# rubund/gnuais

Measured on AMD Instinct MI355X. Metric: Msamples/s demodulated (N-channel batch, full chain), higher is better.
Workload: dtype f32 FIR on int16 samples; u32 PLL/HDLC/CRC; 1 GPU; C3: 16384 ch x 48000 samples @48 kHz per GPU, full chain incl. HDLC/CRC-16; channels_per_gpu=16384, samples_per_channel=48000, parallelism=channels sharded over 1 GPU(s), one process per GPU, no collectives

## Files before the change

gnuais_amd/csrc/hdlc_crc.hip:

```cpp
#include <hip/hip_runtime.h>
#include <stdint.h>

#include "kernels.h"

namespace gnuais {

enum { ST_SKURR = 1, ST_PREAMBLE = 2, ST_STARTSIGN = 3, ST_DATA = 4, ST_STOPSIGN = 5 };

constexpr uint32_t CAND_VALID = 0x10000u;
constexpr int PACK_MAX = PACK_STRIDE;

__global__ void hdlc_reset_kernel(uint32_t *__restrict__ ctl, int N)
{
    const int c = blockIdx.x * blockDim.x + threadIdx.x;
    if (c >= N) return;
    ctl[c] = ST_SKURR;
    ctl[(size_t) N + c] = 0;
    ctl[(size_t) 2 * N + c] = 0;
    ctl[(size_t) 3 * N + c] = 0;
    ctl[(size_t) 4 * N + c] = 0;
    ctl[(size_t) 5 * N + c] = 0;
}

__global__ void hdlc_fsm_reset_kernel(uint32_t *__restrict__ ctl, int N)
{
    const int c = blockIdx.x * blockDim.x + threadIdx.x;
    if (c >= N) return;
    ctl[c] = ST_SKURR;
    ctl[(size_t) N + c] = 0;
    ctl[(size_t) 4 * N + c] = 0;
}

__device__ __forceinline__ uint32_t lowmask(int k)
{
    return k >= 32 ? ~0u : ((1u << k) - 1u);
}
__device__ __forceinline__ int ctz32(uint32_t v)
{
    return v ? __ffs((int) v) - 1 : 32;
}
__device__ __forceinline__ int clz32(uint32_t v)
{
    return v ? __clz((int) v) : 32;
}

__global__ __launch_bounds__(64) __attribute__((amdgpu_waves_per_eu(7, 8))) void hdlc_deframe_kernel(
    const uint32_t *__restrict__ segbits, const uint32_t *__restrict__ segcnt,
    uint32_t *__restrict__ ctl, uint32_t *__restrict__ cand, uint32_t *__restrict__ cand_first,
    uint32_t *__restrict__ cand_count, int32_t *__restrict__ counters,
    uint32_t *__restrict__ flags, int N, int n_seg, int seg_words, int K)
{
    __builtin_amdgcn_s_setprio(3);
    const int cg = blockIdx.x * blockDim.x + threadIdx.x;
    const bool live = cg < N;
    const size_t c = (size_t) (live ? cg : N - 1), n_ = (size_t) N;

    const uint32_t c0 = ctl[c];
    int state = c0 & 7, nstartsign = (c0 >> 3) & 15, antallpreamble = (c0 >> 7) & 15;
    int antallenner = (c0 >> 11) & 7, bitstuff = (c0 >> 14) & 1;
    uint32_t last = (c0 >> 15) & 1;
    int bufferpos = (c0 >> 16) & 511;
    uint32_t cur = ctl[n_ + c];
    const uint32_t seen0 = ctl[2 * n_ + c], seenhi0 = ctl[5 * n_ + c];
    uint32_t nstart = ctl[3 * n_ + c];
    int rawpos = (int) ctl[4 * n_ + c];
    int lost2 = 0;

    const bool open0 = (state == ST_DATA || state == ST_STOPSIGN);
    const uint32_t first = nstart - (open0 ? 1u : 0u);
    uint32_t *rec = cand + ((size_t) c * K + (open0 ? (nstart - 1) % (uint32_t) K : 0u)) * CAND_WORDS;
    bool rec_ok = open0;

    uint32_t seenbase = seen0;

#define HDLC_RESET()                                                                    \
    do { state = ST_SKURR; nstartsign = 0; antallpreamble = 0; antallenner = 0;        \
         last = 0; bitstuff = 0; bufferpos = 0; } while (0)

    extern __shared__ uint32_t lds_pack[];
    const int tpb = (int) blockDim.x, tx = (int) threadIdx.x;
    const uint32_t *__restrict__ rows = segbits + c * (size_t) n_seg * (size_t) PACK_STRIDE;
    uint32_t pf[PACK_MAX];
    int pf_cnt = live ? (int) segcnt[c * (size_t) n_seg] : 0;
#pragma unroll
    for (int q = 0; q < PACK_MAX / 4; ++q) {
        const uint4 v = reinterpret_cast<const uint4 *>(rows)[q];
        pf[4 * q] = v.x; pf[4 * q + 1] = v.y; pf[4 * q + 2] = v.z; pf[4 * q + 3] = v.w;
    }

    for (int seg = 0; seg < n_seg; ++seg) {
        int tile_end = pf_cnt;
        if (tile_end > seg_words * 32) tile_end = seg_words * 32;
#pragma unroll
        for (int q = 0; q < PACK_MAX; ++q) lds_pack[q * tpb + tx] = pf[q];
        lds_pack[PACK_MAX * tpb + tx] = 0;
        if (seg + 1 < n_seg) {
            const uint32_t *__restrict__ nrow = rows + (size_t) (seg + 1) * (size_t) PACK_STRIDE;
            pf_cnt = live ? (int) segcnt[c * (size_t) n_seg + seg + 1] : 0;
#pragma unroll
            for (int q = 0; q < PACK_MAX / 4; ++q) {
                const uint4 v = reinterpret_cast<const uint4 *>(nrow)[q];
                pf[4 * q] = v.x; pf[4 * q + 1] = v.y; pf[4 * q + 2] = v.z; pf[4 * q + 3] = v.w;
            }
        }
        int pos = 0;
#define FETCH_WINDOW()                                                                          \
        const int lw = pos >> 5, sh = pos & 31;                                                 \
        const uint32_t lo = lds_pack[lw * tpb + tx], hi = lds_pack[(lw + 1) * tpb + tx];        \
        const uint32_t W = sh ? ((lo >> sh) | (hi << (32 - sh))) : lo;   \
        const int nv = (tile_end - pos < 32) ? tile_end - pos : 32

        while (__any(pos < tile_end)) {
            while (__any(pos < tile_end && state == ST_SKURR)) {
                if (pos < tile_end && state == ST_SKURR) {
                    FETCH_WINDOW();
                    const uint32_t vm = lowmask(nv);
                    const uint32_t A = W ^ ((W << 1) | last);
                    const uint32_t B2 = A & (A << 1), B4 = B2 & (B2 << 2), B8 = B4 & (B4 << 4);
                    const uint32_t B15 = B8 & (B8 << 7);
                    const int t = ctz32(~A);
                    const int need = 14 - antallpreamble;
                    const uint32_t C = lowmask(t) & ~lowmask(need > 0 ? need : 0);
                    const uint32_t TR = (B15 | C) & ~W & vm;
                    if (TR) {
                        pos += ctz32(TR) + 1;
                        state = ST_PREAMBLE;
                        antallpreamble = 0;
                        last = 0;
                    } else {
                        pos += nv;
                        last = (W >> (nv - 1)) & 1u;
                        const int ap = (t >= nv) ? antallpreamble + nv : clz32(~(A << (32 - nv)));
                        antallpreamble = ap > 15 ? 15 : ap;
                    }
                }
            }
            while (__any(pos < tile_end && state != ST_SKURR && state != ST_DATA)) {
                if (pos < tile_end && state != ST_SKURR && state != ST_DATA) {
                    FETCH_WINDOW();
                    int k = 0;
                    if (state == ST_STOPSIGN) {
                        const uint32_t x = W & 1u;
                        const int nb = bufferpos - 6 - 16;
                        if (x == 0 && nb > 0) {
                            if (rec_ok) {
                                rec[CAND_HDR + (rawpos >> 5)] = cur;
                                const uint32_t eb = seenbase + (uint32_t) pos;
                                const uint32_t ebhi = (seenhi0 + (eb < seen0 ? 1u : 0u)) & 31u;
                                rec[1] = eb;
                                rec[0] = (uint32_t) nb | CAND_VALID | ((uint32_t) rawpos << 17) | (ebhi << 27);
                            }
                        } else {
                            ++lost2;
                            if (rec_ok) {
                                rec[CAND_HDR + (rawpos >> 5)] = cur;
                                rec[0] = (uint32_t) rawpos << 17;
                            }
                        }
                        HDLC_RESET();
                        last = x;
                        k = 1;
                    } else if (state != ST_PREAMBLE && state != ST_STARTSIGN) {
                        HDLC_RESET();
                        last = W & 1u;
                        k = 1;
                    } else {
                        if (state == ST_PREAMBLE && nstartsign == 0) {
                            const uint32_t A = W ^ ((W << 1) | last);
                            int t = ctz32(~A);
                            if (t > nv) t = nv;
                            if (t > 0) {
                                antallpreamble = antallpreamble + t > 15 ? 15 : antallpreamble + t;
                                last = (W >> (t - 1)) & 1u;
                                k = t;
                            }
                            if (k < nv) {
                                const uint32_t x0 = (W >> k) & 1u;
                                nstartsign = x0 ? 3 : 1;
                                last = x0;
                                ++k;
                            }
                        }
                        if (k < nv && nstartsign != 0) {
                            const int R = 7 - nstartsign;
                            const int avail = nv - k;
                            int L = ctz32(~(W >> k));
                            if (L > avail) L = avail;
                            if (L >= R + 1) {
                                HDLC_RESET(); nstartsign = 1; last = 1; k += R + 1;
                            } else if (L < avail) {
                                if (L == R) {
                                    state = ST_DATA; nstartsign = 1; antallenner = 0; antallpreamble = 0;
                                    bufferpos = 0; cur = 0; rawpos = 0; bitstuff = 0; last = 0;
                                    rec_ok = (nstart - first) < (uint32_t) K;
                                    rec = cand + ((size_t) c * K + nstart % (uint32_t) K) * CAND_WORDS;
                                    if (rec_ok) rec[0] = 0; else flags[1] = 1;
                                    ++nstart;
                                } else if (L == R - 1) {
                                    HDLC_RESET(); nstartsign = 1; last = 0;
                                } else {
                                    HDLC_RESET(); last = 0;
                                }
                                k += L + 1;
                            } else {
                                nstartsign += L;
                                if (nstartsign >= 6) { state = ST_STARTSIGN; antallpreamble = 0; }
                                last = 1;
                                k += L;
                            }
                        }
                    }
                    pos += k;
                }
            }
            while (__any(pos < tile_end && state == ST_DATA)) {
                if (pos < tile_end && state == ST_DATA) {
                    FETCH_WINDOW();
                    if (bitstuff) {
                        const uint32_t x = W & 1u;
                        if (x) {
                            state = ST_STOPSIGN;
                        } else {
                            if ((rawpos & 31) == 31) {
                                if (rec_ok) rec[CAND_HDR + (rawpos >> 5)] = cur;
                                cur = 0;
                            }
// ... 9 lines not shown
                        if (nw > 32 - m) nw = 32 - m;
                        if (nw > room) nw = room;
                        const int nvE = nw + m;
                        const uint32_t vmE = lowmask(nvE);
                        const uint32_t E = ((W << m) | lowmask(m)) & vmE;
                        const uint32_t X1 = E & (E >> 1), X2 = X1 & (X1 >> 2);
                        const uint32_t R5 = X2 & (E >> 4);
                        const uint32_t S5 = R5 & ~(E << 1);
                        const uint32_t P5 = S5 << 4;
                        const uint32_t nx = E >> 1, kn = vmE >> 1;
                        const uint32_t END5 = P5 & nx & kn;
                        const uint32_t STF5 = P5 & ~nx & kn;
                        const uint32_t PND5 = P5 & ~kn;
                        int nraw, stored;
                        if (END5) {
                            const int pe = ctz32(END5);
                            nraw = pe + 1 - m;
                            stored = nraw - __popc(STF5 & lowmask(pe));
                        } else {
                            nraw = nw;
                            stored = nw - __popc(STF5);
                        }
                        {
                            const uint32_t sb = W & lowmask(nraw);
                            const int bsh = rawpos & 31;
                            const uint64_t t64 = (uint64_t) sb << bsh;
                            cur |= (uint32_t) t64;
                            if (bsh + nraw >= 32) {
                                if (rec_ok) rec[CAND_HDR + (rawpos >> 5)] = cur;
                                cur = (uint32_t) (t64 >> 32);
                            }
                            rawpos += nraw;
                        }
                        bufferpos += stored;
                        if (END5) {
                            pos += nraw + 1;
                            state = ST_STOPSIGN;
                            antallenner = 0;
                            last = 1;
                        } else {
                            pos += nraw;
                            const uint32_t xl = (W >> (nraw - 1)) & 1u;
                            if (bufferpos >= 449) {
                                if (rec_ok) rec[0] = 0;
                                HDLC_RESET();
                                last = xl;
                            } else if (PND5) {
                                bitstuff = 1;
                                antallenner = 0;
                                last = 1;
                            } else {
                                const int r = clz32(~(E << (32 - nvE)));
                                last = xl;
                                antallenner = r > 0 ? r - 1 : 0;
                            }
                        }
                    }
                }
            }
        }
#undef FETCH_WINDOW
        seenbase += (uint32_t) tile_end;
    }
#undef HDLC_RESET

    if (live) {
        ctl[c] = (uint32_t) state | ((uint32_t) nstartsign << 3) | ((uint32_t) antallpreamble << 7) |
                 ((uint32_t) antallenner << 11) | ((uint32_t) bitstuff << 14) | (last << 15) |
                 ((uint32_t) bufferpos << 16);
        ctl[n_ + c] = cur;
        ctl[2 * n_ + c] = seenbase;
        ctl[5 * n_ + c] = seenhi0 + (seenbase < seen0 ? 1u : 0u);
        ctl[3 * n_ + c] = nstart;
        ctl[4 * n_ + c] = (uint32_t) rawpos;
        const bool open1 = (state == ST_DATA || state == ST_STOPSIGN);
        const uint32_t limit = nstart - (open1 ? 1u : 0u);
        cand_first[c] = first;
        uint32_t cnt = limit - first;
        cand_count[c] = cnt > (uint32_t) K ? (uint32_t) K : cnt;
        if (lost2) counters[2 * n_ + c] += lost2;
    }
}

__global__ __launch_bounds__(256) void hdlc_crc_kernel(
    const uint32_t *__restrict__ cand, const uint32_t *__restrict__ cand_first,
    const uint32_t *__restrict__ cand_count, int32_t *__restrict__ counters,
    uint32_t *__restrict__ frames, uint32_t *__restrict__ flags, uint32_t frame_cap, int N, int K,
    uint2 *__restrict__ chunks, int n_pass)
{
    __shared__ uint32_t tab[256];
    __shared__ uint32_t pre[K3_CH + 1];
    extern __shared__ uint32_t k3_dyn[];
    uint32_t (*const stage)[HDLC_BUF_WORDS + 1] = reinterpret_cast<uint32_t (*)[HDLC_BUF_WORDS + 1]>(k3_dyn);
    uint32_t (*const rawlds)[CAND_WORDS - CAND_HDR + 1] =
        reinterpret_cast<uint32_t (*)[CAND_WORDS - CAND_HDR + 1]>(k3_dyn + 256 * (HDLC_BUF_WORDS + 1));
    __shared__ uint32_t wave_cnt[4];
    __shared__ uint32_t pass_base;
    const int tid = threadIdx.x;
    const int c_own = blockIdx.x * K3_CH + tid;

    {
        uint32_t t = (uint32_t) tid;
#pragma unroll
        for (int k = 0; k < 8; ++k) t = (t >> 1) ^ ((t & 1u) ? 0x8408u : 0u);
        tab[tid] = t;
    }
    if (tid < K3_CH) pre[tid + 1] = (c_own < N) ? cand_count[c_own] : 0u;
    __syncthreads();
    if (tid == 0) {
        uint32_t run = 0;
        pre[0] = 0;
        for (int q = 1; q <= K3_CH; ++q) { run += pre[q]; pre[q] = run; }
    }
    __syncthreads();
    const uint32_t total = pre[K3_CH];
    const size_t n_ = (size_t) N;

    int pass = 0;
    for (uint32_t i0 = 0; i0 < total; i0 += 256, ++pass) {
        const uint32_t i = i0 + (uint32_t) tid;
        bool good = false;
        uint32_t out[16];
#pragma unroll
        for (int q = 0; q < 16; ++q) out[q] = 0;
        if (i < total) {
            int lo = 0, hi = K3_CH - 1;
            while (lo < hi) {
                const int mid = (lo + hi + 1) >> 1;
                if (pre[mid] <= i) lo = mid; else hi = mid - 1;
            }
            const int c = blockIdx.x * K3_CH + lo;
            const uint32_t j = i - pre[lo];
            const uint32_t slot = (cand_first[c] + j) % (uint32_t) K;
            const uint32_t *rec = cand + ((size_t) c * K + slot) * CAND_WORDS;
            const uint32_t hdr = rec[0];
            if (hdr & CAND_VALID) {
                const int n = (int) (hdr & 0xffffu);
                const int rawlen = (int) ((hdr >> 17) & 0x3ffu);
                const int nbytes = n >> 3, buflen = nbytes + 2;
                {
                    uint32_t raw[CAND_WORDS - CAND_HDR];
#pragma unroll
                    for (int q = 0; q < CAND_WORDS - CAND_HDR; ++q) raw[q] = rec[CAND_HDR + q];
#pragma unroll
                    for (int q = 0; q < CAND_WORDS - CAND_HDR; ++q) rawlds[tid][q] = raw[q];
                    unsigned long long acc = 0;
                    uint32_t prevw = 0;
                    int fill = 0, ow = 0;
                    const int nwords = (rawlen + 31) >> 5;
#pragma unroll 1
                    for (int q = 0; q < nwords; ++q) {
                        uint32_t rw = rawlds[tid][q];
                        const int nvq = rawlen - 32 * q < 32 ? rawlen - 32 * q : 32;
                        const unsigned long long cc = ((unsigned long long) rw << 32) | prevw;
                        const uint32_t five = (uint32_t) (cc >> 31) & (uint32_t) (cc >> 30) & (uint32_t) (cc >> 29) &
                                              (uint32_t) (cc >> 28) & (uint32_t) (cc >> 27);
                        uint32_t stf = five & ~rw & (nvq >= 32 ? ~0u : (1u << nvq) - 1u);
                        prevw = rw;
                        int nout = nvq;
                        while (stf) {
                            const int pz = 31 - __clz((int) stf);
                            stf &= ~(1u << pz);
                            rw = (rw & ((1u << pz) - 1u)) | ((pz >= 31 ? 0u : rw >> (pz + 1)) << pz);
                            --nout;
                        }
                        if (nout < 32) rw &= (1u << nout) - 1u;
                        acc |= (unsigned long long) rw << fill;
                        fill += nout;
                        if (fill >= 32) {
                            if (ow <= HDLC_BUF_WORDS) stage[tid][ow] = (uint32_t) acc;
                            ++ow;
                            acc >>= 32;
                            fill -= 32;
                        }
                    }
                    if (ow <= HDLC_BUF_WORDS) stage[tid][ow] = (uint32_t) acc;
                    for (int q = ow + 1; q <= HDLC_BUF_WORDS; ++q) stage[tid][q] = 0;
                }
                uint32_t w[HDLC_BUF_WORDS];
#pragma unroll
                for (int q = 0; q < HDLC_BUF_WORDS; ++q) w[q] = stage[tid][q];
                uint32_t crc = 0xffffu;
#pragma unroll
                for (int q = 0; q < HDLC_BUF_WORDS; ++q) {
#pragma unroll
                    for (int bq = 0; bq < 4; ++bq) {
                        if (q * 4 + bq < buflen) {
                            const uint32_t byte = (w[q] >> (8 * bq)) & 0xffu;
                            crc = (crc >> 8) ^ tab[(crc ^ byte) & 0xffu];
                        }
                    }
                }
                if (crc == 0xf0b8u) {
                    good = true;
                    atomicAdd(&counters[c], 1);
                    out[0] = (uint32_t) c;
                    out[1] = rec[1];
#pragma unroll
                    for (int q = 0; q < 14; ++q) {
                        uint32_t v = 0;
                        if (q * 4 < nbytes) {
                            v = w[q];
                            const int keep = nbytes - q * 4;
                            if (keep < 4) v &= (1u << (8 * keep)) - 1u;
                        }
                        if (q == 13) v = (v & 0xffu) | ((1u | ((hdr >> 27) << 1)) << 8) | ((uint32_t) n << 16);
                        out[2 + q] = v;
                    }
                } else {
                    atomicAdd(&counters[n_ + c], 1);
                }
            }
        }
        const unsigned long long m = __ballot(good);
        const int wave = tid >> 6, lane = tid & 63;
        const uint32_t below = (uint32_t) __popcll(m & ((1ull << lane) - 1ull));
        if (lane == 0) wave_cnt[wave] = (uint32_t) __popcll(m);
        __syncthreads();
        uint32_t woff = 0, npass = 0;
#pragma unroll
        for (int q = 0; q < 4; ++q) {
            if (q < wave) woff += wave_cnt[q];
            npass += wave_cnt[q];
        }
        if (tid == 0) {
            const uint32_t base = npass ? atomicAdd(&flags[0], npass) : 0u;
            pass_base = base;
            if (chunks && pass < n_pass)
                chunks[(size_t) blockIdx.x * n_pass + pass] =
                    make_uint2(base, base >= frame_cap ? 0u : (npass < frame_cap - base ? npass : frame_cap - base));
        }
        __syncthreads();
        if (good) {
            const uint32_t idx = pass_base + woff + below;
            if (idx < frame_cap) {
                uint4 *dst = reinterpret_cast<uint4 *>(frames + (size_t) idx * 16);
                dst[0] = make_uint4(out[0], out[1], out[2], out[3]);
                dst[1] = make_uint4(out[4], out[5], out[6], out[7]);
                dst[2] = make_uint4(out[8], out[9], out[10], out[11]);
                dst[3] = make_uint4(out[12], out[13], out[14], out[15]);
            } else {
                flags[1] = 1;
            }
        }
        __syncthreads();
    }
    if (chunks)
        for (int q = pass + tid; q < n_pass; q += 256) chunks[(size_t) blockIdx.x * n_pass + q] = make_uint2(0u, 0u);
}

hipError_t launch_hdlc_deframe(const HdlcLaunch &a, hipStream_t stream)
{
    const int lpw = a.lanes_per_wave > 0 ? a.lanes_per_wave : 64;
    if (a.seg_words > PACK_MAX) return hipErrorInvalidValue;
    hipLaunchKernelGGL(hdlc_deframe_kernel, dim3((a.N + lpw - 1) / lpw), dim3(lpw),
                       (PACK_MAX + 1) * lpw * sizeof(uint32_t), stream,
                       a.segbits, a.segcnt, a.ctl, a.cand, a.cand_first, a.cand_count, a.counters,
                       a.frame_count, a.N, a.n_seg, a.seg_words, a.K);
    return hipGetLastError();
}

hipError_t launch_hdlc_crc(const HdlcLaunch &a, hipStream_t stream)
{
    constexpr size_t K3_DYN_LDS = 256 * ((HDLC_BUF_WORDS + 1) + (CAND_WORDS - CAND_HDR + 1)) * sizeof(uint32_t);
    hipLaunchKernelGGL(hdlc_crc_kernel, dim3((unsigned) ((a.N + K3_CH - 1) / K3_CH)), dim3(256), K3_DYN_LDS,
                       stream, a.cand, a.cand_first, a.cand_count, a.counters,
                       (uint32_t *) a.frames, a.frame_count, a.frame_cap, a.N, a.K, a.chunks, k3_passes(a.K_call > 0 ? a.K_call : a.K));
    return hipGetLastError();
}

hipError_t launch_hdlc_fsm_reset(uint32_t *ctl, int N, hipStream_t stream)
{
    hipLaunchKernelGGL(hdlc_fsm_reset_kernel, dim3((N + 255) / 256), dim3(256), 0, stream, ctl, N);
    return hipGetLastError();
}

hipError_t launch_hdlc_reset(uint32_t *ctl, int N, hipStream_t stream)
{
    hipLaunchKernelGGL(hdlc_reset_kernel, dim3((N + 255) / 256), dim3(256), 0, stream, ctl, N);
    return hipGetLastError();
}

}
```

gnuais_amd/csrc/hdlc_events.hip:

```cpp
#include <hip/hip_runtime.h>
#include <stdint.h>

#include "kernels.h"

namespace gnuais {

namespace {

enum { ST_SKURR = 1, ST_PREAMBLE = 2, ST_STARTSIGN = 3, ST_DATA = 4, ST_STOPSIGN = 5 };
constexpr uint32_t CAND_VALID = 0x10000u;
constexpr int EW = PACK_STRIDE;
constexpr int NONE = 1 << 20;

__device__ __forceinline__ uint32_t lowmask(int k) { return k >= 32 ? ~0u : k <= 0 ? 0u : ((1u << k) - 1u); }
__device__ __forceinline__ int ctz32(uint32_t v) { return v ? __ffs((int) v) - 1 : 32; }
__device__ __forceinline__ int clz32(uint32_t v) { return v ? __clz((int) v) : 32; }
__device__ __forceinline__ int wave_max_i(int v, int lanes, int lane)
{
#pragma unroll
    for (int o = 32; o; o >>= 1) {
        const int u = __shfl_xor(v, o);
        v = ((lane ^ o) < lanes && u > v) ? u : v;
    }
    return v;
}

}

constexpr int EV_ROWS = (EW + 2) + 4 * EW + (EW + 1);

template <int TPB>
__global__ __launch_bounds__(64) void hdlc_events_kernel(
    const uint32_t *__restrict__ segbits, const uint32_t *__restrict__ segcnt,
    uint32_t *__restrict__ ctl, uint32_t *__restrict__ cand, uint32_t *__restrict__ cand_first,
    uint32_t *__restrict__ cand_count, int32_t *__restrict__ counters,
    uint32_t *__restrict__ flags, int N, int n_seg, int seg_words, int K)
{
    __builtin_amdgcn_s_setprio(3);
    extern __shared__ uint32_t lds[];
    const int tpb = TPB > 0 ? TPB : (int) blockDim.x, tx = (int) threadIdx.x;
    const int cg = blockIdx.x * blockDim.x + threadIdx.x;
    const bool live = cg < N;
    const size_t c = (size_t) (live ? cg : N - 1), n_ = (size_t) N;
    uint32_t *const Xa = lds + tx, *const NAa = Xa + (EW + 2) * tpb, *const CBa = NAa + EW * tpb,
                   *const E6a = CBa + EW * tpb, *const SFa = E6a + EW * tpb, *const PSa = SFa + EW * tpb;
#define XW(q) Xa[((q) + 1) * tpb]

    const uint32_t c0 = ctl[c];
    int state = c0 & 7, nstartsign = (c0 >> 3) & 15, antallpreamble = (c0 >> 7) & 15;
    int antallenner = (c0 >> 11) & 7, bitstuff = (c0 >> 14) & 1;
    uint32_t last = (c0 >> 15) & 1;
    int bufferpos = (c0 >> 16) & 511;
    uint32_t cur = ctl[n_ + c];
    const uint32_t seen0 = ctl[2 * n_ + c], seenhi0 = ctl[5 * n_ + c];
    uint32_t nstart = ctl[3 * n_ + c];
    int rawpos = (int) ctl[4 * n_ + c];
    int lost2 = 0;

    const bool open0 = (state == ST_DATA || state == ST_STOPSIGN);
    const uint32_t first = nstart - (open0 ? 1u : 0u);
    uint32_t *rec = cand + ((size_t) c * K + (open0 ? (nstart - 1) % (uint32_t) K : 0u)) * CAND_WORDS;
    bool rec_ok = open0;
    uint32_t seenbase = seen0;

#define HDLC_RESET()                                                                    \
    do { state = ST_SKURR; nstartsign = 0; antallpreamble = 0; antallenner = 0;        \
         last = 0; bitstuff = 0; bufferpos = 0; } while (0)
#define ENTER_DATA()                                                                    \
    do { state = ST_DATA; nstartsign = 1; antallenner = 0; antallpreamble = 0;         \
         bufferpos = 0; cur = 0; rawpos = 0; bitstuff = 0; last = 0;                    \
         rec_ok = (nstart - first) < (uint32_t) K;                                      \
         rec = cand + ((size_t) c * K + nstart % (uint32_t) K) * CAND_WORDS;            \
         if (rec_ok) rec[0] = 0; else flags[1] = 1;                                     \
         ++nstart; } while (0)
#define RAW_APPEND(v_, n_bits_)                                                         \
    do { const uint32_t sb_ = (v_); const int nb_ = (n_bits_), bsh_ = rawpos & 31;      \
         const uint64_t t64_ = (uint64_t) sb_ << bsh_;                                  \
         cur |= (uint32_t) t64_;                                                        \
         if (bsh_ + nb_ >= 32) {                                                        \
             if (rec_ok) rec[CAND_HDR + (rawpos >> 5)] = cur;                           \
             cur = (uint32_t) (t64_ >> 32);                                             \
         }                                                                              \
         rawpos += nb_; } while (0)
#define STOP_BIT(x_, at_)                                                               \
    do { const int nb_ = bufferpos - 6 - 16;                                            \
         if ((x_) == 0 && nb_ > 0) {                                                    \
             if (rec_ok) {                                                              \
                 const uint32_t eb_ = seenbase + (uint32_t) (at_);                      \
                 const uint32_t ebhi_ = (seenhi0 + (eb_ < seen0 ? 1u : 0u)) & 31u;      \
                 rec[CAND_HDR + (rawpos >> 5)] = cur;                                   \
                 rec[1] = eb_;                                                          \
                 rec[0] = (uint32_t) nb_ | CAND_VALID | ((uint32_t) rawpos << 17) | (ebhi_ << 27); \
             }                                                                          \
         } else {                                                                       \
             ++lost2;                                                                   \
             if (rec_ok) {       \
                 rec[CAND_HDR + (rawpos >> 5)] = cur;                                   \
                 rec[0] = (uint32_t) rawpos << 17;                                      \
             }                                                                          \
         }                                                                              \
         HDLC_RESET();                                                                  \
         last = (x_); } while (0)

    auto slow_bit = [&](uint32_t x, int at) {
        int ns_v = nstartsign, bp_v = bufferpos;
        {
        int nstartsign = ns_v, bufferpos = bp_v;
        switch (state) {
        case ST_DATA:
            if (bitstuff) {
                if (x == 1) {
                    state = ST_STOPSIGN;
                } else {
                    RAW_APPEND(0u, 1);
                }
                bitstuff = 0;
            } else {
                if (x == last && x == 1) {
                    if (++antallenner == 4) { bitstuff = 1; antallenner = 0; }
                } else {
                    antallenner = 0;
                }
                RAW_APPEND(x, 1);
                if (++bufferpos >= 449) {
                    if (rec_ok) rec[0] = 0;
                    HDLC_RESET();
                }
            }
            break;
        case ST_SKURR:
            antallpreamble = (x != last) ? (antallpreamble < 15 ? antallpreamble + 1 : 15) : 0;
            if (antallpreamble > 14 && x == 0) { state = ST_PREAMBLE; antallpreamble = 0; }
            break;
        case ST_PREAMBLE:
            if (x != last && nstartsign == 0) {
                antallpreamble = antallpreamble < 15 ? antallpreamble + 1 : 15;
            } else if (x == 1) {
                if (nstartsign == 0) nstartsign = 3;
                else if (nstartsign == 5) { nstartsign = 6; antallpreamble = 0; state = ST_STARTSIGN; }
                else ++nstartsign;
            } else {
                if (nstartsign == 0) nstartsign = 1; else HDLC_RESET();
            }
            break;
        case ST_STARTSIGN:
            if (nstartsign >= 7) {
                if (x == 0) { ENTER_DATA(); nstartsign = 0; } else HDLC_RESET();
            } else if (x == 0) {
                HDLC_RESET();
            }
            ++nstartsign;
            if (nstartsign > 15) nstartsign = 15;
            break;
        case ST_STOPSIGN:
            STOP_BIT(x, at);
            break;
        default:
            HDLC_RESET();
            break;
        }
        ns_v = nstartsign; bp_v = bufferpos;
        }
        nstartsign = ns_v; bufferpos = bp_v;
        last = x;
    };

    const uint32_t *__restrict__ rows = segbits + c * (size_t) n_seg * (size_t) PACK_STRIDE;
    uint32_t pf[EW];
    int pf_cnt = 0;
    bool pf_ready = false;
    auto fetch = [&](int seg) {
        const uint32_t *__restrict__ row = rows + (size_t) seg * (size_t) PACK_STRIDE;
        {
            pf_cnt = live ? (int) segcnt[c * (size_t) n_seg + seg] : 0;
#pragma unroll
            for (int q = 0; q < EW / 4; ++q) {
                const uint4 v = reinterpret_cast<const uint4 *>(row)[q];
                pf[4 * q] = v.x; pf[4 * q + 1] = v.y; pf[4 * q + 2] = v.z; pf[4 * q + 3] = v.w;
            }
        }
        pf_ready = true;
    };

    for (int seg = 0; seg < n_seg; ++seg) {
        if (!pf_ready) fetch(seg);
        int tile_end = pf_cnt;
        if (tile_end > seg_words * 32) tile_end = seg_words * 32;

        const int m_in = (state == ST_DATA) ? (bitstuff ? 5 : (last ? antallenner + 1 : 0)) : 0;
        uint32_t prevw = (state == ST_DATA) ? (m_in ? ~0u << (32 - m_in) : 0u) : (last << 31);
        uint32_t ps = 0, nzNA = 0, nzCB = 0, nzE6 = 0;
        XW(-1) = prevw;
#pragma unroll
        for (int q = 0; q < EW; ++q) XW(q) = pf[q];
        pf_ready = false;
        if (seg + 1 < n_seg) fetch(seg + 1);
        const int nwq = __builtin_amdgcn_readfirstlane((int) wave_max_i((tile_end + 31) >> 5, tpb, tx));
        auto shl_in = [](uint32_t v, uint32_t below, int n) -> uint32_t {
            return __builtin_amdgcn_alignbit(v, below, 32 - n);
        };
        uint32_t pA = 0, pa2 = 0, pa4 = 0, pa8 = 0;
        uint32_t pu2 = prevw & (prevw << 1);
        uint32_t pt = (pu2 & (pu2 << 2)) & (prevw << 4);
#pragma unroll
        for (int q = 0; q < EW; ++q) {
            if (q >= nwq) {
                XW(q) = 0; NAa[q * tpb] = 0; CBa[q * tpb] = 0; E6a[q * tpb] = 0; SFa[q * tpb] = 0; PSa[q * tpb] = ps;
                continue;
            }
            const uint32_t vm = lowmask(tile_end - 32 * q);
            const uint32_t xw = XW(q) & vm;
            const uint32_t A = (xw ^ shl_in(xw, prevw, 1)) & vm;
            const uint32_t a2 = A & shl_in(A, pA, 1), a4 = a2 & shl_in(a2, pa2, 2), a8 = a4 & shl_in(a4, pa4, 4);
            const uint32_t a15 = a8 & shl_in(a8, pa8, 7);
            const uint32_t u2 = xw & shl_in(xw, prevw, 1), u4 = u2 & shl_in(u2, pu2, 2);
            const uint32_t t5 = u4 & shl_in(xw, prevw, 4);
            const uint32_t na = ~A & vm, cb = a15 & ~xw & vm;
            const uint32_t e6 = u4 & shl_in(u2, pu2, 4) & vm;
            const uint32_t sf = shl_in(t5, pt, 1) & ~xw & vm;
            XW(q) = xw;
            NAa[q * tpb] = na;
            CBa[q * tpb] = cb;
            E6a[q * tpb] = e6;
            SFa[q * tpb] = sf;
            PSa[q * tpb] = ps;
            ps += (uint32_t) __popc(sf);
            nzNA |= (na < 1u ? na : 1u) << q;
            nzCB |= (cb < 1u ? cb : 1u) << q;
            nzE6 |= (e6 < 1u ? e6 : 1u) << q;
            pA = A; pa2 = a2; pa4 = a4; pa8 = a8; pu2 = u2; pt = t5;
            prevw = xw;
        }
        XW(EW) = 0;
        PSa[EW * tpb] = ps;

        auto first_set = [&](const uint32_t *arr, uint32_t nz, int p) -> int {
            if (p >= tile_end) return NONE;
            const int q = p >> 5;
            const uint32_t m = arr[q * tpb] & (~0u << (p & 31));
            if (m) return 32 * q + ctz32(m);
            const uint32_t rest = q >= 31 ? 0u : nz & (~0u << (q + 1));
            if (!rest) return NONE;
            const int q2 = ctz32(rest);
            return 32 * q2 + ctz32(arr[q2 * tpb]);
        };
        auto bit_at = [&](int p) -> uint32_t { return (XW(p >> 5) >> (p & 31)) & 1u; };
        auto window = [&](int p) -> uint32_t {
            const int q = p >> 5, sh = p & 31;
            const uint32_t lo = XW(q), hi = XW(q + 1 <= EW ? q + 1 : EW);
            return sh ? ((lo >> sh) | (hi << (32 - sh))) : lo;
        };
        auto stuffed = [&](int a, int b) -> int {
            if (b <= a) return 0;
            const int qa = a >> 5, qb = b >> 5;
            int n = (int) PSa[qb * tpb] - (int) PSa[qa * tpb];
            n -= __popc(SFa[qa * tpb] & lowmask(a & 31));
            if (qb < EW) n += __popc(SFa[qb * tpb] & lowmask(b & 31));
            return n;
        };

        int pos = 0;
        int rs = -1;
        bool hunt0 = true;
        bool slow = false;

        auto hunt = [&]() {
            int trig = NONE;
            if (rs < 0 && hunt0) {
                const int t0 = first_set(NAa, nzNA, 0);
                int k0 = 14 - antallpreamble;
                if (k0 < 0) k0 = 0;
                const int lim = t0 < tile_end ? t0 : tile_end;
                if (k0 < lim && bit_at(k0)) ++k0;
                if (k0 < lim) trig = k0;
                const int cb = first_set(CBa, nzCB, 0);
                if (cb < trig) trig = cb;
            } else {
                const int from = rs + 15 > pos ? rs + 15 : pos;
                trig = first_set(CBa, nzCB, from);
            }
            if (trig < tile_end) {
                state = ST_PREAMBLE;
                antallpreamble = 0;
                last = 0;
                pos = trig + 1;
            } else {
                int lastna = -1;
                for (uint32_t nz = nzNA; nz;) {
                    const int q = 31 - clz32(nz);
                    const uint32_t m = NAa[q * tpb];
                    lastna = 32 * q + 31 - clz32(m);
                    break;
                }
                int ap;
                if (rs < 0 && hunt0) ap = lastna < 0 ? antallpreamble + tile_end : tile_end - 1 - lastna;
                else {
                    const int since = tile_end - 1 - rs, run = tile_end - 1 - lastna;
                    ap = since < run ? since : run;
                }
                antallpreamble = ap > 15 ? 15 : ap;
                last = bit_at(tile_end - 1);
                pos = tile_end;
            }
        };

        while (__any(pos < tile_end)) {
            if (pos < tile_end) {
                if (state == ST_SKURR && !slow) hunt();
                if (state == ST_PREAMBLE && nstartsign == 0 && pos < tile_end && !slow) {
                    const int j = first_set(NAa, nzNA, pos);
                    if (j >= tile_end) {
                        const int ap = antallpreamble + (tile_end - pos);
                        antallpreamble = ap > 15 ? 15 : ap;
                        last = bit_at(tile_end - 1);
                        pos = tile_end;
                    } else {
                        const int ap = antallpreamble + (j - pos);
                        antallpreamble = ap > 15 ? 15 : ap;
                        const uint32_t xj = bit_at(j);
                        nstartsign = xj ? 3 : 1;
                        last = xj;
                        pos = j + 1;
                    }
                }
                if (((state == ST_PREAMBLE && nstartsign != 0) || state == ST_STARTSIGN) && pos < tile_end && !slow) {
                    const uint32_t W = window(pos);
                    const int avail = tile_end - pos < 32 ? tile_end - pos : 32;
                    const int R = 7 - nstartsign;
                    int Lr = ctz32(~W);
                    if (Lr > avail) Lr = avail;
                    if (R < 0) {
                        slow = true;
                    } else if (Lr >= R + 1) {
                        HDLC_RESET(); nstartsign = 1; last = 1;
                        rs = pos + R; hunt0 = false;
                        pos += R + 1;
                    } else if (Lr < avail) {
                        if (Lr == R) {
                            ENTER_DATA();
                            pos += Lr + 1;
                        } else if (Lr == R - 1) {
                            HDLC_RESET(); nstartsign = 1; last = 0;
                            rs = pos + Lr; hunt0 = false;
                            pos += Lr + 1;
                        } else {
                            HDLC_RESET(); last = 0;
                            rs = pos + Lr; hunt0 = false;
                            pos += Lr + 1;
                        }
                    } else {
                        nstartsign += Lr;
                        if (nstartsign >= 6) { state = ST_STARTSIGN; antallpreamble = 0; }
                        last = 1;
                        pos += Lr;
                    }
                }
                if (state == ST_DATA && pos < tile_end && !slow) {
                    const int e6 = first_set(E6a, nzE6, pos);
                    const int e = e6 < tile_end ? e6 : tile_end;
                    const int stored = (e - pos) - stuffed(pos, e);
                    if (bufferpos + stored >= 449) {
                        int need = 449 - bufferpos, p = pos, t = pos;
                        for (;;) {
                            const int q = p >> 5;
                            const int we = (32 * (q + 1) < e) ? 32 * (q + 1) : e;
                            uint32_t m = ~SFa[q * tpb] & (~0u << (p & 31)) & lowmask(we - 32 * q);
                            const int n = __popc(m);
                            if (n >= need) {
                                for (int k = 1; k < need; ++k) m &= m - 1;
                                t = 32 * q + ctz32(m);
                                break;
                            }
                            need -= n;
                            p = we;
                        }
                        if (rec_ok) rec[0] = 0;
                        const uint32_t xt = bit_at(t);
                        HDLC_RESET();
                        last = xt;
                        rs = t; hunt0 = false;
                        pos = t + 1;
                    } else {
                        for (int p = pos; p < e;) {
                            const int sh = p & 31;
                            const int take = (32 - sh < e - p) ? 32 - sh : e - p;
                            RAW_APPEND((XW(p >> 5) >> sh) & lowmask(take), take);
                            p += take;
                        }
                        bufferpos += stored;
                        if (e6 < tile_end) {
                            state = ST_STOPSIGN;
                            antallenner = 0;
                            bitstuff = 0;
                            last = 1;
                            pos = e6 + 1;
                        } else {
                            int r;
                            if (tile_end >= 8) {
                                r = clz32(~(window(tile_end - 8) << 24));
                            } else {
                                r = clz32(~((XW(0) << (32 - tile_end)) | (XW(-1) >> tile_end)));
                            }
                            last = bit_at(tile_end - 1);
                            if (r >= 5) { bitstuff = 1; antallenner = 0; }
                            else { bitstuff = 0; antallenner = r > 0 ? r - 1 : 0; }
                            pos = tile_end;
                        }
                    }
                }
                if (state == ST_STOPSIGN && pos < tile_end && !slow) {
                    const uint32_t x = bit_at(pos);
                    STOP_BIT(x, pos);
                    rs = pos; hunt0 = false;
                    pos += 1;
                }
                if (pos < tile_end && (slow || state < ST_SKURR || state > ST_STOPSIGN)) {
                    const int st0 = state;
                    const uint32_t x = bit_at(pos);
                    slow_bit(x, pos);
                    if (state == ST_SKURR && st0 != ST_SKURR) { rs = pos; hunt0 = false; }
                    if (state != st0) slow = false;
                    pos += 1;
                }
                if (state == ST_SKURR && !slow && pos < tile_end) hunt();
            }
        }
        seenbase += (uint32_t) tile_end;
    }
#undef XW
#undef HDLC_RESET
#undef ENTER_DATA
#undef RAW_APPEND
#undef STOP_BIT

    if (live) {
        ctl[c] = (uint32_t) state | ((uint32_t) nstartsign << 3) | ((uint32_t) antallpreamble << 7) |
                 ((uint32_t) antallenner << 11) | ((uint32_t) bitstuff << 14) | (last << 15) |
                 ((uint32_t) bufferpos << 16);
        ctl[n_ + c] = cur;
        ctl[2 * n_ + c] = seenbase;
        ctl[5 * n_ + c] = seenhi0 + (seenbase < seen0 ? 1u : 0u);
        ctl[3 * n_ + c] = nstart;
        ctl[4 * n_ + c] = (uint32_t) rawpos;
        const bool open1 = (state == ST_DATA || state == ST_STOPSIGN);
        const uint32_t limit = nstart - (open1 ? 1u : 0u);
        cand_first[c] = first;
        uint32_t cnt = limit - first;
        cand_count[c] = cnt > (uint32_t) K ? (uint32_t) K : cnt;
        if (lost2) counters[2 * n_ + c] += lost2;
    }
}

hipError_t launch_hdlc_events(const HdlcLaunch &a, hipStream_t stream)
{
    if (a.seg_words > PACK_STRIDE) return hipErrorInvalidValue;
    const int lpw = a.lanes_per_wave >= 1 && a.lanes_per_wave <= 64 ? a.lanes_per_wave : 64;
    const dim3 grid((a.N + lpw - 1) / lpw), block(lpw);
    const size_t lds = EV_ROWS * lpw * sizeof(uint32_t);
#define EV_LAUNCH(T)                                                                                                  \
    hipLaunchKernelGGL(hdlc_events_kernel<T>, grid, block, lds, stream, a.segbits, a.segcnt, a.ctl, a.cand, a.cand_first, \
                       a.cand_count, a.counters, a.frame_count, a.N, a.n_seg, a.seg_words, a.K)
    switch (lpw) {
    case 8: EV_LAUNCH(8); break;
    case 16: EV_LAUNCH(16); break;
    case 32: EV_LAUNCH(32); break;
    case 64: EV_LAUNCH(64); break;
    default: EV_LAUNCH(0); break;
    }
#undef EV_LAUNCH
    return hipGetLastError();
}

}
```

gnuais_amd/csrc/kernels.h:

```cpp
#pragma once
#include <hip/hip_runtime.h>
#include <stdint.h>

#include "fir_plan.h"

namespace gnuais {

struct FirLaunch : FirThresholds {
    const int16_t *x;
    const int16_t *hist;
    uint32_t *sgn;
    float *dump;
    int *maxval;
    int16_t *hist_out;
    int *maxval_next;
    const float *d_taps;
    float te[64];
    int N, L;
    int NT, NE, d;
    float ctaps[48];
    const float *te_mem;
    int map;
    int max_segments = 0;
    const struct MfmaTaps *mfma = nullptr;
};
int launch_fir_sign_quantum(int NC);
hipError_t launch_fir_sign(const FirLaunch &a, hipStream_t stream);
int launch_fir_sign_pk_quantum(int NC);
struct alignas(16) MfmaTaps { int a[3][3][64][4]; int k0; };
void fir_sign_mfma_pack(const int *tq48, long tq_sum, MfmaTaps *out);
hipError_t launch_fir_sign_mfma(const FirLaunch &a, int first, hipStream_t stream);
hipError_t launch_fir_sign_pk(const FirLaunch &a, hipStream_t stream);
hipError_t launch_fir_generic(const FirLaunch &a, hipStream_t stream);
hipError_t launch_fir_history(const int16_t *x, const int16_t *hist_in, int16_t *hist_out,
                              int N, int L, int NT, hipStream_t stream);

constexpr int PLL_LDS_BYTES = 81 * 1024;
constexpr int SEG_WORDS = 64;
constexpr int SEG_LEN = SEG_WORDS * 32;
constexpr int PACK_STRIDE = 16;
__host__ __device__ inline size_t sgn_index(int w, int N, int c)
{
    return ((size_t) (w >> 2) * (size_t) N + (size_t) c) * 4 + (size_t) (w & 3);
}
__host__ __device__ inline size_t sgn_words_alloc(int W, int N)
{
    return (size_t) ((W + 3) / 4 + 1) * 4 * (size_t) N;
}
struct PllLaunch {
    const uint32_t *sgn;
    uint32_t *pll;
    uint32_t *prev;
    uint32_t *lastbit;
    uint32_t *watchdog;
    uint32_t *segbits;
    uint32_t *segcnt;
    int N, L, n_seg, seg_words;
    uint32_t pllinc;
    int n_cu;
    int variant = 0;
};
int pll_form_of(const PllLaunch &a);
int pll_need_lds();
hipError_t pll_prepare_device();
hipError_t launch_pll(const PllLaunch &a, hipStream_t stream);
bool pll_tp_applicable(const PllLaunch &a);
hipError_t launch_pll_tp(const PllLaunch &a, hipStream_t stream);
constexpr int PLL_TP_MAX_CHANNELS = 1536;

constexpr int HDLC_CTL_WORDS = 6;
constexpr int HDLC_BUF_WORDS = 15;
constexpr int CAND_HDR = 2;
constexpr int CAND_WORDS = 20;
struct HdlcLaunch {
    const uint32_t *segbits;
    const uint32_t *segcnt;
    uint32_t *ctl;
    uint32_t *cand;
    uint32_t *cand_first;
    uint32_t *cand_count;
    int32_t *counters;
    void *frames;
    uint32_t *frame_count;
    uint32_t frame_cap;
    int N, n_seg, seg_words, K;
    int K_call = 0;
    int lanes_per_wave;
    uint2 *chunks = nullptr;
};
constexpr int K3_CH = 32;
inline int k3_blocks(int N) { return (N + K3_CH - 1) / K3_CH; }
inline int k3_passes(int K) { return (K3_CH * K + 255) / 256; }
hipError_t launch_hdlc_deframe(const HdlcLaunch &a, hipStream_t stream);
hipError_t launch_hdlc_events(const HdlcLaunch &a, hipStream_t stream);
hipError_t launch_hdlc_crc(const HdlcLaunch &a, hipStream_t stream);
hipError_t launch_hdlc_reset(uint32_t *ctl, int N, hipStream_t stream);
hipError_t launch_hdlc_fsm_reset(uint32_t *ctl, int N, hipStream_t stream);

struct FrameTimeLaunch {
    const void *frames;
    const uint32_t *frame_count;
    uint32_t frame_cap;
    const uint32_t *ctl;
    const uint32_t *segcnt;
    int64_t *times;
    int N, n_seg, seg_words;
    int len;
    int64_t n0;
};
hipError_t launch_frame_times(const FrameTimeLaunch &a, hipStream_t stream);
hipError_t launch_frame_times_gather(const int64_t *times, const uint32_t *order, int n, int64_t *out, hipStream_t stream);

hipError_t launch_iq_power(const int16_t *iq, uint32_t *carry, int64_t *ring, int RB, int N, int len,
                           unsigned long long n0, bool first, hipStream_t stream);
struct FrameSignalLaunch {
    const void *frames;
    const uint32_t *frame_count;
    uint32_t frame_cap;
    const int64_t *times;
    const int64_t *ring;
    void *signal;
    int RB, N;
    int len;
    int64_t n0;
    uint32_t pllinc;
    int n_taps, afc_window;
    int64_t v0;
};
hipError_t launch_frame_signal(const FrameSignalLaunch &a, hipStream_t stream);

hipError_t launch_occ_code(const int64_t *sums, int RB, uint16_t *codes, int CB, int N, long long j0, int count,
                           hipStream_t stream);
struct OccCoverLaunch {
    const void *frames;
    const uint32_t *frame_count;
    uint32_t frame_cap;
    const int64_t *times;
    uint8_t *cover;
    int CB, N;
    int len;
    int64_t n0;
    uint32_t pllinc;
    int n_taps, afc_window;
    int64_t v0, b0;
};
hipError_t launch_occ_cover(const OccCoverLaunch &a, hipStream_t stream);
struct OccEpochLaunch {
    uint16_t *codes;
    uint8_t *cover;
    uint8_t *carry;
    void *out;
    int CB, N, E, margin;
    int64_t first;
    bool first_epoch;
};
hipError_t launch_occ_epoch(const OccEpochLaunch &a, hipStream_t stream);
// ... 159 lines not shown
```

Before: 1.647 million Msamples/s.

## Defer raw-bit capture from HDLC event FSM to CRC kernel via span marks

```diff
diff --git a/gnuais_amd/csrc/hdlc_crc.hip b/gnuais_amd/csrc/hdlc_crc.hip
--- a/gnuais_amd/csrc/hdlc_crc.hip
+++ b/gnuais_amd/csrc/hdlc_crc.hip
@@ -77,7 +77,7 @@
     do { state = ST_SKURR; nstartsign = 0; antallpreamble = 0; antallenner = 0;        \
          last = 0; bitstuff = 0; bufferpos = 0; } while (0)
 
-    extern __shared__ uint32_t lds_pack[];
+    GNUAIS_DYN_SHARED(uint32_t, lds_pack);
     const int tpb = (int) blockDim.x, tx = (int) threadIdx.x;
     const uint32_t *__restrict__ rows = segbits + c * (size_t) n_seg * (size_t) PACK_STRIDE;
     uint32_t pf[PACK_MAX];
@@ -142,6 +142,7 @@
                     if (state == ST_STOPSIGN) {
                         const uint32_t x = W & 1u;
                         const int nb = bufferpos - 6 - 16;
+                        if (rec_ok) rec[CAND_MARK] = 0;
                         if (x == 0 && nb > 0) {
                             if (rec_ok) {
                                 rec[CAND_HDR + (rawpos >> 5)] = cur;
@@ -317,15 +318,61 @@
     }
 }
 
+__device__ __forceinline__ void k3_gather(uint32_t *raw, uint32_t *pk, uint32_t *rec, uint32_t mark, int rawlen,
+                                          const uint32_t *__restrict__ segbits, const uint32_t *__restrict__ segcnt,
+                                          size_t c, int n_seg, int seg_words)
+{
+    int P = (int) ((mark >> 21) & 0x3ffu), seg = (int) ((mark >> 10) & 0x7ffu), bit = (int) (mark & 0x3ffu);
+    if (rawlen > 32 * CAND_RAW_WORDS - 1) rawlen = 32 * CAND_RAW_WORDS - 1;
+    if (P > rawlen) P = rawlen;
+    int ow = P >> 5, fill = P & 31, rem = rawlen - P;
+    unsigned long long acc = fill ? (raw[ow] & ((1u << fill) - 1u)) : 0u;
+    const int cap = seg_words * 32;
+    const uint32_t *cnts = segcnt + c * (size_t) n_seg;
+    const uint4 *row = reinterpret_cast<const uint4 *>(segbits + (c * (size_t) n_seg + (size_t) seg) * PACK_STRIDE);
+    while (rem > 0 && seg < n_seg) {
+        const uint4 v0 = row[0], v1 = row[1], v2 = row[2], v3 = row[3];
+        const int cnt = (int) cnts[seg];
+        const int cnt_now = cnt < cap ? cnt : cap;
+        pk[0] = v0.x; pk[1] = v0.y; pk[2] = v0.z; pk[3] = v0.w; pk[4] = v1.x; pk[5] = v1.y; pk[6] = v1.z; pk[7] = v1.w;
+        pk[8] = v2.x; pk[9] = v2.y; pk[10] = v2.z; pk[11] = v2.w; pk[12] = v3.x; pk[13] = v3.y; pk[14] = v3.z; pk[15] = v3.w;
+        ++seg;
+        row += PACK_STRIDE / 4;
+#pragma unroll 1
+        for (int p = bit; p < cnt_now && rem > 0;) {
+            const int sh = p & 31;
+            int take = 32 - sh;
+            if (take > cnt_now - p) take = cnt_now - p;
+            if (take > rem) take = rem;
+            const uint32_t v = (pk[p >> 5] >> sh) & (take >= 32 ? ~0u : (1u << take) - 1u);
+            acc |= (unsigned long long) v << fill;
+            fill += take;
+            if (fill >= 32) {
+                raw[ow++] = (uint32_t) acc;
+                acc >>= 32;
+                fill -= 32;
+            }
+            p += take;
+            rem -= take;
+        }
+        bit = 0;
+    }
+    raw[ow] = (uint32_t) acc;
+#pragma unroll 1
+    for (int q = P >> 5; q <= ow; ++q) rec[CAND_HDR + q] = raw[q];
+    rec[CAND_MARK] = 0;
+}
+
 __global__ __launch_bounds__(256) void hdlc_crc_kernel(
-    const uint32_t *__restrict__ cand, const uint32_t *__restrict__ cand_first,
+    uint32_t *__restrict__ cand, const uint32_t *__restrict__ cand_first,
     const uint32_t *__restrict__ cand_count, int32_t *__restrict__ counters,
     uint32_t *__restrict__ frames, uint32_t *__restrict__ flags, uint32_t frame_cap, int N, int K,
-    uint2 *__restrict__ chunks, int n_pass)
+    uint2 *__restrict__ chunks, int n_pass,
+    const uint32_t *__restrict__ segbits, const uint32_t *__restrict__ segcnt, int n_seg, int seg_words)
 {
     __shared__ uint32_t tab[256];
     __shared__ uint32_t pre[K3_CH + 1];
-    extern __shared__ uint32_t k3_dyn[];
+    GNUAIS_DYN_SHARED(uint32_t, k3_dyn);
     uint32_t (*const stage)[HDLC_BUF_WORDS + 1] = reinterpret_cast<uint32_t (*)[HDLC_BUF_WORDS + 1]>(k3_dyn);
     uint32_t (*const rawlds)[CAND_WORDS - CAND_HDR + 1] =
         reinterpret_cast<uint32_t (*)[CAND_WORDS - CAND_HDR + 1]>(k3_dyn + 256 * (HDLC_BUF_WORDS + 1));
@@ -367,18 +414,23 @@
             const int c = blockIdx.x * K3_CH + lo;
             const uint32_t j = i - pre[lo];
             const uint32_t slot = (cand_first[c] + j) % (uint32_t) K;
-            const uint32_t *rec = cand + ((size_t) c * K + slot) * CAND_WORDS;
+            uint32_t *rec = cand + ((size_t) c * K + slot) * CAND_WORDS;
             const uint32_t hdr = rec[0];
+            const int rawlen = (int) ((hdr >> 17) & 0x3ffu);
+            if (rawlen > 0) {
+                uint32_t raw[CAND_WORDS - CAND_HDR];
+#pragma unroll
+                for (int q = 0; q < CAND_WORDS - CAND_HDR; ++q) raw[q] = rec[CAND_HDR + q];
+#pragma unroll
+                for (int q = 0; q < CAND_WORDS - CAND_HDR; ++q) rawlds[tid][q] = raw[q];
+                const uint32_t mark = raw[CAND_MARK - CAND_HDR];
+                if (mark & CAND_SPAN)
+                    k3_gather(rawlds[tid], stage[tid], rec, mark, rawlen, segbits, segcnt, (size_t) c, n_seg, seg_words);
+            }
             if (hdr & CAND_VALID) {
                 const int n = (int) (hdr & 0xffffu);
-                const int rawlen = (int) ((hdr >> 17) & 0x3ffu);
                 const int nbytes = n >> 3, buflen = nbytes + 2;
                 {
-                    uint32_t raw[CAND_WORDS - CAND_HDR];
-#pragma unroll
-                    for (int q = 0; q < CAND_WORDS - CAND_HDR; ++q) raw[q] = rec[CAND_HDR + q];
-#pragma unroll
-                    for (int q = 0; q < CAND_WORDS - CAND_HDR; ++q) rawlds[tid][q] = raw[q];
                     unsigned long long acc = 0;
                     uint32_t prevw = 0;
                     int fill = 0, ow = 0;
@@ -498,9 +550,12 @@
 hipError_t launch_hdlc_crc(const HdlcLaunch &a, hipStream_t stream)
 {
     constexpr size_t K3_DYN_LDS = 256 * ((HDLC_BUF_WORDS + 1) + (CAND_WORDS - CAND_HDR + 1)) * sizeof(uint32_t);
+    static_assert(HDLC_BUF_WORDS + 1 >= PACK_STRIDE, "k3_gather parks a pack in the thread's stage row");
+    if (a.seg_words > PACK_STRIDE) return hipErrorInvalidValue;
     hipLaunchKernelGGL(hdlc_crc_kernel, dim3((unsigned) ((a.N + K3_CH - 1) / K3_CH)), dim3(256), K3_DYN_LDS,
                        stream, a.cand, a.cand_first, a.cand_count, a.counters,
-                       (uint32_t *) a.frames, a.frame_count, a.frame_cap, a.N, a.K, a.chunks, k3_passes(a.K_call > 0 ? a.K_call : a.K));
+                       (uint32_t *) a.frames, a.frame_count, a.frame_cap, a.N, a.K, a.chunks, k3_passes(a.K_call > 0 ? a.K_call : a.K),
+                       a.segbits, a.segcnt, a.n_seg, a.seg_words);
     return hipGetLastError();
 }
 
diff --git a/gnuais_amd/csrc/hdlc_events.hip b/gnuais_amd/csrc/hdlc_events.hip
--- a/gnuais_amd/csrc/hdlc_events.hip
+++ b/gnuais_amd/csrc/hdlc_events.hip
@@ -37,7 +37,7 @@
     uint32_t *__restrict__ flags, int N, int n_seg, int seg_words, int K)
 {
     __builtin_amdgcn_s_setprio(3);
-    extern __shared__ uint32_t lds[];
+    GNUAIS_DYN_SHARED(uint32_t, lds);
     const int tpb = TPB > 0 ? TPB : (int) blockDim.x, tx = (int) threadIdx.x;
     const int cg = blockIdx.x * blockDim.x + threadIdx.x;
     const bool live = cg < N;
@@ -51,10 +51,8 @@
     int antallenner = (c0 >> 11) & 7, bitstuff = (c0 >> 14) & 1;
     uint32_t last = (c0 >> 15) & 1;
     int bufferpos = (c0 >> 16) & 511;
-    uint32_t cur = ctl[n_ + c];
     const uint32_t seen0 = ctl[2 * n_ + c], seenhi0 = ctl[5 * n_ + c];
     uint32_t nstart = ctl[3 * n_ + c];
-    int rawpos = (int) ctl[4 * n_ + c];
     int lost2 = 0;
 
     const bool open0 = (state == ST_DATA || state == ST_STOPSIGN);
@@ -62,58 +60,56 @@
     uint32_t *rec = cand + ((size_t) c * K + (open0 ? (nstart - 1) % (uint32_t) K : 0u)) * CAND_WORDS;
     bool rec_ok = open0;
     uint32_t seenbase = seen0;
+    uint32_t fmark = 0, rbase = 0;
+    if (open0) {
+        uint32_t p0 = ctl[4 * n_ + c];
+        if (p0 > 32u * CAND_RAW_WORDS - 1u) p0 = 32u * CAND_RAW_WORDS - 1u;
+        fmark = p0 << 21;
+        rbase = p0 - seen0 + (state == ST_STOPSIGN ? 1u : 0u);
+        if (live) rec[CAND_HDR + (p0 >> 5)] = ctl[n_ + c];
+    }
 
 #define HDLC_RESET()                                                                    \
     do { state = ST_SKURR; nstartsign = 0; antallpreamble = 0; antallenner = 0;        \
          last = 0; bitstuff = 0; bufferpos = 0; } while (0)
-#define ENTER_DATA()                                                                    \
+#define ENTER_DATA(first_)                                                              \
     do { state = ST_DATA; nstartsign = 1; antallenner = 0; antallpreamble = 0;         \
-         bufferpos = 0; cur = 0; rawpos = 0; bitstuff = 0; last = 0;                    \
+         bufferpos = 0; bitstuff = 0; last = 0;                                         \
+         fmark = ((uint32_t) seg << 10) | (uint32_t) (first_);                          \
+         rbase = 0u - (seenbase + (uint32_t) (first_));                                 \
          rec_ok = (nstart - first) < (uint32_t) K;                                      \
          rec = cand + ((size_t) c * K + nstart % (uint32_t) K) * CAND_WORDS;            \
          if (rec_ok) rec[0] = 0; else flags[1] = 1;                                     \
          ++nstart; } while (0)
-#define RAW_APPEND(v_, n_bits_)                                                         \
-    do { const uint32_t sb_ = (v_); const int nb_ = (n_bits_), bsh_ = rawpos & 31;      \
-         const uint64_t t64_ = (uint64_t) sb_ << bsh_;                                  \
-         cur |= (uint32_t) t64_;                                                        \
-         if (bsh_ + nb_ >= 32) {                                                        \
-             if (rec_ok) rec[CAND_HDR + (rawpos >> 5)] = cur;                           \
-             cur = (uint32_t) (t64_ >> 32);                                             \
-         }                                                                              \
-         rawpos += nb_; } while (0)
 #define STOP_BIT(x_, at_)                                                               \
     do { const int nb_ = bufferpos - 6 - 16;                                            \
+         const uint32_t eb_ = seenbase + (uint32_t) (at_);                              \
+         const uint32_t rawlen_ = (rbase + eb_ - 1u) & 0x3ffu;                          \
          if ((x_) == 0 && nb_ > 0) {                                                    \
              if (rec_ok) {                                                              \
-                 const uint32_t eb_ = seenbase + (uint32_t) (at_);                      \
                  const uint32_t ebhi_ = (seenhi0 + (eb_ < seen0 ? 1u : 0u)) & 31u;      \
-                 rec[CAND_HDR + (rawpos >> 5)] = cur;                                   \
+                 rec[CAND_MARK] = CAND_SPAN | fmark;                                    \
                  rec[1] = eb_;                                                          \
-                 rec[0] = (uint32_t) nb_ | CAND_VALID | ((uint32_t) rawpos << 17) | (ebhi_ << 27); \
+                 rec[0] = (uint32_t) nb_ | CAND_VALID | (rawlen_ << 17) | (ebhi_ << 27); \
              }                                                                          \
          } else {                                                                       \
              ++lost2;                                                                   \
              if (rec_ok) {       \
-                 rec[CAND_HDR + (rawpos >> 5)] = cur;                                   \
-                 rec[0] = (uint32_t) rawpos << 17;                                      \
+                 rec[CAND_MARK] = CAND_SPAN | fmark;                                    \
+                 rec[0] = rawlen_ << 17;                                                \
              }                                                                          \
          }                                                                              \
          HDLC_RESET();                                                                  \
          last = (x_); } while (0)
 
-    auto slow_bit = [&](uint32_t x, int at) {
+    auto slow_bit = [&](uint32_t x, int at, int seg) {
         int ns_v = nstartsign, bp_v = bufferpos;
         {
         int nstartsign = ns_v, bufferpos = bp_v;
         switch (state) {
         case ST_DATA:
             if (bitstuff) {
-                if (x == 1) {
-                    state = ST_STOPSIGN;
-                } else {
-                    RAW_APPEND(0u, 1);
-                }
+                if (x == 1) state = ST_STOPSIGN;
                 bitstuff = 0;
             } else {
                 if (x == last && x == 1) {
@@ -121,7 +117,6 @@
                 } else {
                     antallenner = 0;
                 }
-                RAW_APPEND(x, 1);
                 if (++bufferpos >= 449) {
                     if (rec_ok) rec[0] = 0;
                     HDLC_RESET();
@@ -145,7 +140,7 @@
             break;
         case ST_STARTSIGN:
             if (nstartsign >= 7) {
-                if (x == 0) { ENTER_DATA(); nstartsign = 0; } else HDLC_RESET();
+                if (x == 0) { ENTER_DATA(at + 1); nstartsign = 0; } else HDLC_RESET();
             } else if (x == 0) {
                 HDLC_RESET();
             }
@@ -182,10 +177,12 @@
         pf_ready = true;
     };
 
+    int last_end = 0;
     for (int seg = 0; seg < n_seg; ++seg) {
         if (!pf_ready) fetch(seg);
         int tile_end = pf_cnt;
         if (tile_end > seg_words * 32) tile_end = seg_words * 32;
+        last_end = tile_end;
 
         const int m_in = (state == ST_DATA) ? (bitstuff ? 5 : (last ? antallenner + 1 : 0)) : 0;
         uint32_t prevw = (state == ST_DATA) ? (m_in ? ~0u << (32 - m_in) : 0u) : (last << 31);
@@ -337,7 +334,7 @@
                         pos += R + 1;
                     } else if (Lr < avail) {
                         if (Lr == R) {
-                            ENTER_DATA();
+                            ENTER_DATA(pos + Lr + 1);
                             pos += Lr + 1;
                         } else if (Lr == R - 1) {
                             HDLC_RESET(); nstartsign = 1; last = 0;
@@ -381,12 +378,6 @@
                         rs = t; hunt0 = false;
                         pos = t + 1;
                     } else {
-                        for (int p = pos; p < e;) {
-                            const int sh = p & 31;
-                            const int take = (32 - sh < e - p) ? 32 - sh : e - p;
-                            RAW_APPEND((XW(p >> 5) >> sh) & lowmask(take), take);
-                            p += take;
-                        }
                         bufferpos += stored;
                         if (e6 < tile_end) {
                             state = ST_STOPSIGN;
@@ -417,7 +408,7 @@
                 if (pos < tile_end && (slow || state < ST_SKURR || state > ST_STOPSIGN)) {
                     const int st0 = state;
                     const uint32_t x = bit_at(pos);
-                    slow_bit(x, pos);
+                    slow_bit(x, pos, seg);
                     if (state == ST_SKURR && st0 != ST_SKURR) { rs = pos; hunt0 = false; }
                     if (state != st0) slow = false;
                     pos += 1;
@@ -426,11 +417,52 @@
             }
         }
         seenbase += (uint32_t) tile_end;
+    }
+
+    const bool open1 = live && (state == ST_DATA || state == ST_STOPSIGN);
+    uint32_t cur = 0;
+    int rawpos = 0;
+    {
+        const int P = (int) (fmark >> 21), s0 = (int) ((fmark >> 10) & 0x7ffu), b0 = (int) (fmark & 0x3ffu);
+        int rem = 0;
+        if (open1) {
+            rawpos = P;
+            rem = (int) (rbase + seenbase) - (state == ST_STOPSIGN ? 1 : 0) - P;
+            if (rem > 32 * CAND_RAW_WORDS - 1 - P) rem = 32 * CAND_RAW_WORDS - 1 - P;
+            if (P) cur = ctl[n_ + c];
+        }
+        auto take_bits = [&](const uint32_t *W, int p, int cnt) {
+            while (p < cnt && rem > 0) {
+                const int sh = p & 31, bsh = rawpos & 31;
+                int take = 32 - sh;
+                if (take > cnt - p) take = cnt - p;
+                if (take > rem) take = rem;
+                const uint64_t t64 = (uint64_t) ((W[(p >> 5) * tpb] >> sh) & lowmask(take)) << bsh;
+                cur |= (uint32_t) t64;
+                if (bsh + take >= 32) {
+                    if (rec_ok) rec[CAND_HDR + (rawpos >> 5)] = cur;
+                    cur = (uint32_t) (t64 >> 32);
+                }
+                rawpos += take; p += take; rem -= take;
+            }
+        };
+        const int s_lo = __builtin_amdgcn_readfirstlane(-(int) wave_max_i(-(rem > 0 ? s0 : n_seg), tpb, tx));
+        pf_ready = false;
+        for (int s = s_lo; s < n_seg - 1; ++s) {
+            if (!pf_ready) fetch(s);
+            int cnt = pf_cnt;
+            if (cnt > seg_words * 32) cnt = seg_words * 32;
+#pragma unroll
+            for (int q = 0; q < EW; ++q) NAa[q * tpb] = pf[q];
+            pf_ready = false;
+            if (s + 1 < n_seg - 1) fetch(s + 1);
+            if (s >= s0) take_bits(NAa, s == s0 ? b0 : 0, cnt);
+        }
+        if (n_seg - 1 >= s0) take_bits(Xa + tpb, n_seg - 1 == s0 ? b0 : 0, last_end);
     }
 #undef XW
 #undef HDLC_RESET
 #undef ENTER_DATA
-#undef RAW_APPEND
 #undef STOP_BIT
 
     if (live) {
@@ -453,7 +485,7 @@
 
 hipError_t launch_hdlc_events(const HdlcLaunch &a, hipStream_t stream)
 {
-    if (a.seg_words > PACK_STRIDE) return hipErrorInvalidValue;
+    if (a.seg_words > PACK_STRIDE || a.n_seg > CAND_MARK_PACKS) return hipErrorInvalidValue;
     const int lpw = a.lanes_per_wave >= 1 && a.lanes_per_wave <= 64 ? a.lanes_per_wave : 64;
     const dim3 grid((a.N + lpw - 1) / lpw), block(lpw);
     const size_t lds = EV_ROWS * lpw * sizeof(uint32_t);
diff --git a/gnuais_amd/csrc/kernels.h b/gnuais_amd/csrc/kernels.h
--- a/gnuais_amd/csrc/kernels.h
+++ b/gnuais_amd/csrc/kernels.h
@@ -3,6 +3,10 @@
 #include <stdint.h>
 
 #include "fir_plan.h"
+
+#ifndef GNUAIS_DYN_SHARED
+#define GNUAIS_DYN_SHARED(type, name) extern __shared__ type name[]
+#endif
 
 namespace gnuais {
 
@@ -72,6 +76,10 @@
 constexpr int HDLC_BUF_WORDS = 15;
 constexpr int CAND_HDR = 2;
 constexpr int CAND_WORDS = 20;
+constexpr int CAND_MARK = CAND_WORDS - 1;
+constexpr int CAND_MARK_PACKS = 2048;
+constexpr int CAND_RAW_WORDS = 17;
+constexpr uint32_t CAND_SPAN = 0x80000000u;
 struct HdlcLaunch {
     const uint32_t *segbits;
     const uint32_t *segcnt;
```

New measurement: 1.701 million Msamples/s, median of 6. 1.03x the previous value.
